# yanzq95/DHD

Hardware: AMD Instinct MI355X
Metric: samples/sec (6-cam fwd+bwd) DHD-S view-transform hot path (higher is better)
Workload: dtype f32

## Files before the change

### dhd_amd/csrc/sfa_gemm_cu.h

```cpp
#pragma once
#include "sfa_math.h"
#include "sfa_mfma.h"

namespace dhd_sfa {

constexpr int kCuPatchPitch = 36;

__device__ __forceinline__ void cu_lds_barrier() { asm volatile("s_waitcnt lgkmcnt(0)\n\ts_barrier" ::: "memory"); }

constexpr int cu_swz_c(int p) { return ((((p >> 2) & 7) ^ (p & 1)) | (((p >> 1) & 1) << 3)); }
__host__ __device__ inline int cu_swz(int p) { return ((((p >> 2) & 7) ^ (p & 1)) | (((p >> 1) & 1) << 3)); }

inline size_t cu_lds_bytes(int c, int waves, int nb, bool blend = false) {
  return (size_t)2 * 2 * 32 * 2 * c + (size_t)waves * 32 * kCuPatchPitch * sizeof(float) + ((size_t)nb * 3 + 1) * c * sizeof(float) +
         (blend ? ((size_t)nb + 2) * c * sizeof(float) : 0);
}
inline int cu_max_batch(int c, int waves, bool blend = false) {
  return (int)((160 * 1024 - cu_lds_bytes(c, waves, 0, blend)) / ((size_t)(blend ? 4 : 3) * c * sizeof(float)));
}

struct CuBlend {
  const void* x;
  const float* a1;
  const float* scsh;
// ... 232 lines not shown
        return;
      }
#pragma unroll
      for (int mt = 0; mt < MT; ++mt) {
        if (NACC == 2) {
          acc2[mt] = mfma_bf16(wm[ks][mt], bh, ks == 0 ? zero : acc2[mt]);
          acc[mt] = mfma_bf16(wh[ks][mt], bh, ks == 0 ? zero : acc[mt]);
          acc2[mt] = mfma_bf16(wh[ks][mt], bm, acc2[mt]);
        } else {
          acc[mt] = mfma_bf16(wm[ks][mt], bh, ks == 0 ? zero : acc[mt]);
          acc[mt] = mfma_bf16(wh[ks][mt], bm, acc[mt]);
          acc[mt] = mfma_bf16(wh[ks][mt], bh, acc[mt]);
        }
      }
    });
    stamp(0);
    if (PP) cu_lds_barrier();
    auto next_tile = [&]() {
    stage(std::integral_constant<int, SN>{}, (PAR ^ 1) ^ grp, t + (1 + grp) * t_step);
    stamp(1);
    issue(std::integral_constant<int, SN>{}, t + (1 + grp + R) * t_step);
    stamp(2);
    };
    auto epilogue = [&]() {
    const __amdgpu_buffer_rsrc_t ry =
        __builtin_amdgcn_make_buffer_rsrc(y + (size_t)b * C * hw, 0, (unsigned)((size_t)C * hw * sizeof(float)), 0x00020000);
    const bool quad_ok = live && p0 + 4 * q < hw;
    const int voff_st = quad_ok ? st_voff : 0x7ffffff0;
    if (ABL & 4) {
#pragma unroll
      for (int mt = 0; mt < MT; ++mt)
#pragma unroll
        for (int v = 0; v < 16; ++v) abl_sink += acc[mt][v] + (NACC == 2 ? acc2[mt][v] : 0.f);
    }
#pragma unroll
    for (int mt = 0; mt < ((ABL & 4) ? 0 : MT); ++mt) {
#pragma unroll
      for (int v = 0; v < 16; ++v)
        patch[(8 * (v >> 2) + 4 * h + (v & 3)) * kCuPatchPitch + n] = NACC == 2 ? acc[mt][v] + acc2[mt][v] : acc[mt][v];
#pragma unroll
      for (int k = 0; k < 4; ++k) {
        f32x4 o = *reinterpret_cast<const f32x4*>(patch + (g + 8 * k) * kCuPatchPitch + 4 * q);
        if (EPI == 0) {
          const float s1 = (o.x + o.y) + (o.z + o.w), s2 = (o.x * o.x + o.y * o.y) + (o.z * o.z + o.w * o.w);
          ws1[mt][k] += quad_ok ? s1 : 0.f;
          ws2[mt][k] += quad_ok ? s2 : 0.f;
          const float bs = bias_lds[kbase + 32 * mt + g + 8 * k];
          o.x += bs; o.y += bs; o.z += bs; o.w += bs;
        }
        if (EPI == 1) {
          const int w4 = (int)(mask_r[mt][k] >> (4 * (g & 3)));
#pragma unroll
          for (int e = 0; e < 4; ++e) o[e] = __int_as_float(__float_as_int(o[e]) & __builtin_amdgcn_sbfe(w4, e, 1));
        }
        const int soff = (32 * mt + 8 * k) * row_bytes + p0 * 4;
        if (EPI == 3) {
          const int ch = kbase + 32 * mt + g + 8 * k;
          const float bs = bias_lds[ch];
          o.x += bs; o.y += bs; o.z += bs; o.w += bs;
          const float a = bl_a[b * C + ch], na = 1.0f - a, sc = bl_sc[ch], sh = bl_sc[C + ch];
          const f32x4 pb = xb[mt][k], pv = xv[mt][k];
          f32x4 r;
#pragma unroll
          for (int j = 0; j < 4; ++j) {
            r[j] = blend_out(blend_gate(sc, o[j], sh), a, na, pb[j], pv[j]);
          }
          const __amdgpu_buffer_rsrc_t ro = __builtin_amdgcn_make_buffer_rsrc(
              static_cast<TO*>(bl.out) + (size_t)b * C * hw, 0, (unsigned)((size_t)C * hw * sizeof(TO)), 0x00020000);
          if constexpr (std::is_same_v<TO, float>) {
            store_b128_guarded<SAUX>(__builtin_bit_cast(u32x4, r), ro, voff_st, soff);
          } else {
            typedef TO t4 __attribute__((ext_vector_type(4)));
            const t4 hv = {(TO)r.x, (TO)r.y, (TO)r.z, (TO)r.w};
            __builtin_amdgcn_raw_buffer_store_b64(__builtin_bit_cast(u32x2, hv), ro, quad_ok ? st_voff >> 1 : 0x7ffffff0, soff >> 1, SAUX);
          }
          continue;
        }
        if (!(ABL & 2)) store_b128_guarded<SAUX>(__builtin_bit_cast(u32x4, o), ry, voff_st, soff);
      }
    }
    };
    if (EORD == 0) { next_tile(); epilogue(); } else { epilogue(); next_tile(); }
    stamp(3);
    cu_lds_barrier();
  };

  if (n_mine > 0) {
    auto fill_stores = [&]() {
      const __amdgpu_buffer_rsrc_t ry = __builtin_amdgcn_make_buffer_rsrc(y, 0, 16, 0x00020000);
#pragma unroll
      for (int i = 0; i < 4 * MT; ++i)
        if (!(ABL & 2)) store_b128_guarded<SAUX>(u32x4{0u, 0u, 0u, 0u}, ry, 0x7ffffff0, 0);
    };
    issue(std::integral_constant<int, 0>{}, t0);
    if (R == 2) {
      issue(std::integral_constant<int, 1 % R>{}, t0 + t_step);
      fill_stores();
    }
    stage(std::integral_constant<int, 0>{}, 0, t0);
    issue(std::integral_constant<int, 0>{}, t0 + R * t_step);
    fill_stores();
    cu_lds_barrier();
    if (PP && grp) {
      stage(std::integral_constant<int, 0>{}, 1, t0 + t_step);
      issue(std::integral_constant<int, 0>{}, t0 + 2 * t_step);
      fill_stores();
      cu_lds_barrier();
    }
    for (int i = 0, t = t0; i < n_mine; i += 2, t += 2 * t_step) {
      tile(std::integral_constant<int, 0>{}, t, true);
      tile(std::integral_constant<int, 1>{}, t + t_step, i + 1 < n_mine);
    }
    if (PP && !grp) cu_lds_barrier();
  }

  if ((ABL & 256) && lane == 0) {
    unsigned* o = reinterpret_cast<unsigned*>(stat_part) + 1024 + ((size_t)blockIdx.x * WAVES + wv) * 8;
    for (int i = 0; i < 6; ++i) o[i] = ph[i];
    o[6] = (unsigned)n_mine;
  }
  if ((ABL & 64) && tid == 0) reinterpret_cast<long long*>(stat_part)[blockIdx.x] = (long long)__builtin_readcyclecounter() - abl_clk0;
  if (EPI == 0 && stat_part != nullptr) {
#pragma unroll
    for (int mt = 0; mt < MT; ++mt)
#pragma unroll
      for (int k = 0; k < 4; ++k) {
        float s1 = ws1[mt][k], s2 = ws2[mt][k];
#pragma unroll
        for (int m = 1; m < 8; m <<= 1) {
          s1 += __shfl_xor(s1, m, DHD_WAVE);
          s2 += __shfl_xor(s2, m, DHD_WAVE);
        }
        if (q == 0) {
          float* row = stat_part + (size_t)blockIdx.x * 2 * C + kbase + 32 * mt + g + 8 * k;
          row[0] = s1;
          row[C] = s2;
        }
      }
  }
}

}
```

### dhd_amd/csrc/sfa_stage.hip

```cpp
#include <stdlib.h>

#include <type_traits>

#include "sfa_gemm_cu.h"
#include "sfa_half.h"
#include "sfa_mfma.h"

using namespace dhd_sfa;

namespace {

constexpr int kEwBlock = 256;
constexpr int kPlaneChunks = 4;
constexpr int kPwBlock = 256;
constexpr int kPwStep = 16;
constexpr int kWgBlock = 512;
constexpr int kWgStride = 33;
constexpr int kWgWorkers = 256;

__device__ __forceinline__ float block_sum(float v, float* sm) {
  v = group_sum(v, DHD_WAVE);
  const int lane = threadIdx.x & 63, wv = threadIdx.x >> 6;
  __syncthreads();
  if (lane == 0) sm[wv] = v;
  __syncthreads();
  float t = 0.f;
  for (int k = 0; k < (int)(blockDim.x / DHD_WAVE); ++k) t += sm[k];
  return t;
}

template <class TS> constexpr bool kHalfStorage = !std::is_same_v<TS, float>;
template <class TS> constexpr bool kStreamAll = kHalfStorage<TS>;
template <class TS> constexpr int kWideInFlight = kHalfStorage<TS> ? 2 : 1;
template <class TS> constexpr bool kFoldPairwise = !kHalfStorage<TS>;

template <int N> __device__ __forceinline__ void chunk_range(int hw, int* lo, int* hi) {
  static_assert(N == 4 || N == 8, "16 bytes of float32 or of a half type");
  const int n = hw >> (N == 8 ? 3 : 2), per = (n + kPlaneChunks - 1) / kPlaneChunks;
  *lo = blockIdx.x * per;
  *hi = min(n, *lo + per);
}

template <class TO, int N> struct IoVec {
  static constexpr bool k16 = N == kVec16<TO>;
  static_assert(k16 || (N == 4 && sizeof(TO) == 2), "16 bytes, or four elements of a half type");
  using raw = std::conditional_t<k16, raw16<TO>, u32x2>;
  static __device__ __forceinline__ raw ld(const TO* base, size_t i) { return __builtin_nontemporal_load(reinterpret_cast<const raw*>(base) + i); }
  static __device__ __forceinline__ void widen(raw w, float* v) {
    if constexpr (k16) {
      widen16<TO>(w, v);
    } else {
      const f32x2 a = Pair<TO>::widen(w.x), b = Pair<TO>::widen(w.y);
      v[0] = a.x; v[1] = a.y; v[2] = b.x; v[3] = b.y;
// ... 40 lines not shown
      body(w, i + kEwBlock);
    }
    if (i < hi) body(load(i), i);
  } else {
    for (; i < hi; i += kEwBlock) body(load(i), i);
  }
}


template <class TS>
__device__ __forceinline__ void plane_mean_block(const TS* __restrict__ x, float* __restrict__ part, int hw, float* sm) {
  constexpr int N = kVec16<TS>;
  using X = Vec16<TS, true>;
  const size_t plane = blockIdx.y;
  const TS* p = x + plane * hw;
  int lo, hi;
  chunk_range<N>(hw, &lo, &hi);
  float a0 = 0.f, a1 = 0.f;
  int i = lo + threadIdx.x;
  for (; i + kEwBlock < hi; i += 2 * kEwBlock) {
    float v[N], w[N];
    X::load(p, i, v);
    X::load(p, (size_t)i + kEwBlock, w);
    a0 += tree_sum<N>(v);
    a1 += tree_sum<N>(w);
  }
  if (i < hi) {
    float v[N];
    X::load(p, i, v);
    a0 += tree_sum<N>(v);
  }
  const float tot = block_sum(a0 + a1, sm);
  if (threadIdx.x == 0) part[plane * kPlaneChunks + blockIdx.x] = tot;
}

__global__ __launch_bounds__(kEwBlock) void plane_mean_kernel(const float* __restrict__ x, float* __restrict__ part, int hw) {
  __shared__ float sm[kEwBlock / DHD_WAVE];
  plane_mean_block(x, part, hw, sm);
}

constexpr int kFcBlock = 1024;
__global__ __launch_bounds__(kFcBlock) void fc_forward_kernel(const float* __restrict__ part, const float* __restrict__ w1,
                                                              const float* __restrict__ b1, const float* __restrict__ w2,
                                                              const float* __restrict__ b2, float* __restrict__ s,
                                                              float* __restrict__ hbuf, float* __restrict__ a,
                                                              float* __restrict__ tab, int c, int r, int hw,
                                                              int* __restrict__ ticks, int n_ticks) {
  extern __shared__ float sh[];
  if (blockIdx.x == 0)
    for (int i = threadIdx.x; i < n_ticks; i += kFcBlock) ticks[i] = 0;
  float* ss = sh;
  float* hh = sh + 2 * c;
  const int b = blockIdx.x, c2 = 2 * c;
  for (int i = threadIdx.x; i < c2; i += kFcBlock) {
    const float* q = part + ((size_t)b * c2 + i) * kPlaneChunks;
    float v = ((q[0] + q[1]) + (q[2] + q[3])) / (float)hw;
    ss[i] = v;
    s[(size_t)b * c2 + i] = v;
  }
  __syncthreads();
  const int lane = threadIdx.x & 63, wv = threadIdx.x >> 6;
  for (int j0 = wv * 4; j0 < r; j0 += 4 * (kFcBlock / DHD_WAVE)) {
    float acc[4] = {0.f, 0.f, 0.f, 0.f};
    for (int i = lane; i < c2; i += DHD_WAVE) {
      const float sv = ss[i];
#pragma unroll
      for (int q = 0; q < 4; ++q)
        if (j0 + q < r) acc[q] = fmaf(w1[(size_t)(j0 + q) * c2 + i], sv, acc[q]);
    }
#pragma unroll
    for (int q = 0; q < 4; ++q) {
      const float t = group_sum(acc[q], DHD_WAVE);
      if (lane == 0 && j0 + q < r) {
        const float v = fmaxf(t + b1[j0 + q], 0.f);
        hh[j0 + q] = v;
        hbuf[(size_t)b * r + j0 + q] = v;
      }
    }
  }
  __syncthreads();
  for (int k = threadIdx.x; k < c; k += kFcBlock) {
    float acc = b2[k];
    if ((r & 3) == 0) {
      const f32x4* wrow = reinterpret_cast<const f32x4*>(w2 + (size_t)k * r);
#pragma unroll 8
      for (int j = 0; j < (r >> 2); ++j) {
        const f32x4 wv4 = wrow[j];
        acc = fmaf(wv4.x, hh[4 * j], acc);
        acc = fmaf(wv4.y, hh[4 * j + 1], acc);
        acc = fmaf(wv4.z, hh[4 * j + 2], acc);
        acc = fmaf(wv4.w, hh[4 * j + 3], acc);
      }
    } else {
      for (int j = 0; j < r; ++j) acc = fmaf(w2[(size_t)k * r + j], hh[j], acc);
    }
    float v = sigmoidf_(acc);
    a[(size_t)b * c + k] = v;
    float* t = tab + (size_t)b * 3 * c;
    t[k] = v;
    t[c + k] = 1.0f - v;
    t[2 * c + k] = 0.f;
  }
}

__global__ __launch_bounds__(kEwBlock) void fc_backward_kernel(const float* __restrict__ da_p1, const float* __restrict__ da_p2,
                                                               const float* __restrict__ a, const float* __restrict__ hbuf,
                                                               const float* __restrict__ w1, const float* __restrict__ w2,
                                                               float* __restrict__ dpre2, float* __restrict__ dh,
                                                               float* __restrict__ ds, int c, int r) {
  extern __shared__ float sh[];
  float* sp = sh;
  float* sd = sh + c;
  const int b = blockIdx.x, c2 = 2 * c;
  for (int k = threadIdx.x; k < c; k += kEwBlock) {
    float g = 0.f;
    for (int q = 0; q < kPlaneChunks; ++q)
      g += da_p1[((size_t)b * kPlaneChunks + q) * c + k] + da_p2[((size_t)b * kPlaneChunks + q) * c + k];
    const float av = a[(size_t)b * c + k];
    const float v = g * av * (1.0f - av);
    sp[k] = v;
    dpre2[(size_t)b * c + k] = v;
  }
  __syncthreads();
  if (r <= kEwBlock && kEwBlock % r == 0) {
    float* pp = sh + c + r;
    const int groups = kEwBlock / r, j = threadIdx.x % r, grp = threadIdx.x / r;
    float acc = 0.f;
#pragma unroll 8
    for (int k = grp; k < c; k += groups) acc = fmaf(w2[(size_t)k * r + j], sp[k], acc);
    pp[grp * r + j] = acc;
    __syncthreads();
    if (threadIdx.x < r) {
      float t = 0.f;
      for (int q = 0; q < groups; ++q) t += pp[q * r + threadIdx.x];
      const float v = hbuf[(size_t)b * r + threadIdx.x] > 0.f ? t : 0.f;
      sd[threadIdx.x] = v;
// ... 125 lines not shown
  scsh[c + ch] = shf;
  for (int b = 0; b < nb; ++b) {
    float* t = tab + (size_t)b * 3 * c;
    t[ch] = sc;
    t[c + ch] = 0.f;
    t[2 * c + ch] = shf;
  }
  if (run_mean) {
    const double unb = n > 1.0 ? var * n / (n - 1.0) : var;
    run_mean[ch] = (float)((1.0 - (double)momentum) * (double)run_mean[ch] + (double)momentum * mu);
    run_var[ch] = (float)((1.0 - (double)momentum) * (double)run_var[ch] + (double)momentum * unb);
  }
}

__device__ __forceinline__ void bn_eval_coef_channel(int ch, const float* __restrict__ gamma, const float* __restrict__ beta,
                                                     const float* __restrict__ run_mean, const float* __restrict__ run_var, float eps,
                                                     float* __restrict__ mean, float* __restrict__ rstd, float* __restrict__ scsh,
                                                     float* __restrict__ tab, int nb, int c) {
  const float rs = 1.0f / sqrtf(run_var[ch] + eps);
  mean[ch] = run_mean[ch];
  rstd[ch] = rs;
  const float sc = gamma[ch] * rs, shf = beta[ch] - run_mean[ch] * sc;
  scsh[ch] = sc;
  scsh[c + ch] = shf;
  for (int b = 0; b < nb; ++b) {
    float* t = tab + (size_t)b * 3 * c;
    t[ch] = sc;
    t[c + ch] = 0.f;
    t[2 * c + ch] = shf;
  }
}

__global__ __launch_bounds__(kEwBlock) void bn_eval_coef_kernel(const float* __restrict__ gamma, const float* __restrict__ beta,
                                                                const float* __restrict__ run_mean, const float* __restrict__ run_var,
                                                                float eps, float* __restrict__ mean, float* __restrict__ rstd,
                                                                float* __restrict__ scsh, float* __restrict__ tab, int nb, int c) {
  const int ch = blockIdx.x * kEwBlock + threadIdx.x;
  if (ch >= c) return;
  bn_eval_coef_channel(ch, gamma, beta, run_mean, run_var, eps, mean, rstd, scsh, tab, nb, c);
}

struct BnEvalJob {
  const float *gamma, *beta, *run_mean, *run_var;
  float eps;
  float *mean, *rstd, *scsh, *tab;
};
__global__ __launch_bounds__(kEwBlock) void bn_eval_coef2_kernel(BnEvalJob j1, BnEvalJob j2, int nb, int c) {
  const int ch = blockIdx.x * kEwBlock + threadIdx.x;
  if (ch >= c) return;
  const BnEvalJob& j = blockIdx.y ? j2 : j1;
  bn_eval_coef_channel(ch, j.gamma, j.beta, j.run_mean, j.run_var, j.eps, j.mean, j.rstd, j.scsh, j.tab, nb, c);
}

template <bool COHERENT>
__device__ __forceinline__ void bn_backward_coef_channel(const float* __restrict__ part, int ch, const float* __restrict__ gamma,
                                                         const float* __restrict__ mean, const float* __restrict__ rstd,
                                                         int training, float* __restrict__ tab, float* __restrict__ dgamma,
                                                         float* __restrict__ dbeta, float* __restrict__ dbias, int nb, int c, int hw,
                                                         double* __restrict__ sums_out, const double* __restrict__ sums_in,
                                                         const double* __restrict__ loc_fwd, const float* __restrict__ shift) {
  double s1 = 0.0, s2 = 0.0;
  if (COHERENT) {
    float v1[16], v2[16];
    for (int q0 = 0; q0 < nb * kPlaneChunks; q0 += 16) {
#pragma unroll
      for (int u = 0; u < 16; ++u) {
        const int q = min(q0 + u, nb * kPlaneChunks - 1);
        v1[u] = __hip_atomic_load(part + ((size_t)q * 2) * c + ch, __ATOMIC_RELAXED, __HIP_MEMORY_SCOPE_AGENT);
        v2[u] = __hip_atomic_load(part + ((size_t)q * 2 + 1) * c + ch, __ATOMIC_RELAXED, __HIP_MEMORY_SCOPE_AGENT);
      }
#pragma unroll
      for (int u = 0; u < 16; ++u)
        if (q0 + u < nb * kPlaneChunks) { s1 += (double)v1[u]; s2 += (double)v2[u]; }
    }
  } else {
    for (int q = 0; q < nb * kPlaneChunks; ++q) {
      s1 += (double)part[((size_t)q * 2) * c + ch];
      s2 += (double)part[((size_t)q * 2 + 1) * c + ch];
    }
  }
  const double n_loc = (double)nb * (double)hw;
  if (sums_out) {
    sums_out[ch] = s1; sums_out[c + ch] = s2;
    if (ch == 0) sums_out[2 * c] = n_loc;
    return;
  }
  const double n = sums_in ? sums_in[2 * c] : n_loc;
  const double g1 = sums_in ? sums_in[ch] : s1, g2 = sums_in ? sums_in[c + ch] : s2;
  const double rs = (double)rstd[ch], mu = (double)mean[ch], ga = (double)gamma[ch];
  if (dgamma) dgamma[ch] = (float)(rs * s2);
  if (dbeta) dbeta[ch] = (float)s1;
  double c0 = ga * rs, c1 = 0.0, c2 = 0.0, db = c0 * s1;
  if (training) {
    c1 = -ga * rs * rs * rs * g2 / n;
    c2 = -ga * rs * g1 / n - c1 * mu;
    db = 0.0;
    if (sums_in) db = c0 * s1 + c1 * (loc_fwd[ch] + n_loc * (double)shift[ch]) + n_loc * c2;
  }
  if (dbias) dbias[ch] = (float)db;
  for (int b = 0; b < nb; ++b) {
    float* t = tab + (size_t)b * 3 * c;
    t[ch] = (float)c0;
    t[c + ch] = (float)c1;
    t[2 * c + ch] = (float)c2;
  }
}

__global__ __launch_bounds__(kEwBlock) void bn_backward_coef_kernel(const float* __restrict__ part, const float* __restrict__ gamma,
                                                                    const float* __restrict__ mean, const float* __restrict__ rstd,
                                                                    int training, float* __restrict__ tab, float* __restrict__ dgamma,
                                                                    float* __restrict__ dbeta, float* __restrict__ dbias, int nb,
                                                                    int c, int hw, double* __restrict__ sums_out,
                                                                    const double* __restrict__ sums_in, const double* __restrict__ loc_fwd,
                                                                    const float* __restrict__ shift) {
  const int ch = blockIdx.x * kEwBlock + threadIdx.x;
  if (ch >= c) return;
  bn_backward_coef_channel<false>(part, ch, gamma, mean, rstd, training, tab, dgamma, dbeta, dbias, nb, c, hw, sums_out, sums_in,
                                  loc_fwd, shift);
}

struct BnTail {
  int* ticket;
  const float* gamma;
  const float* mean;
  const float* rstd;
  float* tab;
  float* dgamma;
  float* dbeta;
  float* dbias;
  int training, nb, hw;
};
__device__ __forceinline__ void bn_backward_publish(const BnTail& t, float* __restrict__ part, size_t q, int ch, int c, float s1,
                                                    float s2) {
  float* p1 = part + (q * 2) * c + ch;
  float* p2 = part + (q * 2 + 1) * c + ch;
  if (t.ticket == nullptr) {
    *p1 = s1;
    *p2 = s2;
    return;
  }
  __hip_atomic_store(p1, s1, __ATOMIC_RELAXED, __HIP_MEMORY_SCOPE_AGENT);
  __hip_atomic_store(p2, s2, __ATOMIC_RELAXED, __HIP_MEMORY_SCOPE_AGENT);
  asm volatile("s_waitcnt vmcnt(0)" ::: "memory");
  if (__hip_atomic_fetch_add(t.ticket + ch, 1, __ATOMIC_RELAXED, __HIP_MEMORY_SCOPE_AGENT) != t.nb * kPlaneChunks - 1) return;
  __hip_atomic_store(t.ticket + ch, 0, __ATOMIC_RELAXED, __HIP_MEMORY_SCOPE_AGENT);
  bn_backward_coef_channel<true>(part, ch, t.gamma, t.mean, t.rstd, t.training, t.tab, t.dgamma, t.dbeta, t.dbias, t.nb, c, t.hw,
                                 nullptr, nullptr, nullptr, nullptr);
}

template <class TS>
__global__ __launch_bounds__(kEwBlock) void pair_sums_kernel(const TS* __restrict__ g, const TS* __restrict__ y,
                                                             const float* __restrict__ mean, float* __restrict__ part, int c, int hw,
                                                             BnTail tail) {
  constexpr int N = kVec16<TS>;
  using Main = Vec16<TS, true>;
  using Tail = Vec16<TS, kStreamAll<TS>>;
  __shared__ float sm[kEwBlock / DHD_WAVE];
  const int plane = blockIdx.y, b = plane / c, ch = plane % c;
  const float mu = mean[ch];
  const TS* gp = g + (size_t)plane * hw;
  const TS* yp = y + (size_t)plane * hw;
  int lo, hi;
  chunk_range<N>(hw, &lo, &hi);
  float s1 = 0.f, s2 = 0.f, t1 = 0.f, t2 = 0.f;
  int i = lo + threadIdx.x;
  for (; i + kEwBlock < hi; i += 2 * kEwBlock) {
    float a[N], v[N], a2[N], v2[N];
    Main::load(gp, i, a);
    Main::load(yp, i, v);
    Main::load(gp, (size_t)i + kEwBlock, a2);
    Main::load(yp, (size_t)i + kEwBlock, v2);
    s1 = fold_sum<TS>(s1, a);
    s2 = fold_dot<TS>(s2, a, [&](int j) { return v[j] - mu; });
    t1 = fold_sum<TS>(t1, a2);
    t2 = fold_dot<TS>(t2, a2, [&](int j) { return v2[j] - mu; });
  }
  if (i < hi) {
    float a[N], v[N];
    Tail::load(gp, i, a);
    Tail::load(yp, i, v);
    s1 = fold_sum<TS>(s1, a);
    s2 = fold_dot<TS>(s2, a, [&](int j) { return v[j] - mu; });
  }
  s1 = block_sum(s1 + t1, sm);
  s2 = block_sum(s2 + t2, sm);
  if (threadIdx.x == 0) bn_backward_publish(tail, part, (size_t)(b * kPlaneChunks + blockIdx.x), ch, c, s1, s2);
}


template <class TS, class TO>
__global__ __launch_bounds__(kEwBlock) void blend2_bn_kernel(const TS* __restrict__ x, const float* __restrict__ a1,
                                                             const TS* __restrict__ y2, const float* __restrict__ scsh,
                                                             TO* __restrict__ out, int c, int hw) {
  constexpr int N = kVec16<TS>;
  using X = Vec16<TS, true>;
  using Y2 = Vec16<TS, kStreamAll<TS>>;
  const int plane = blockIdx.y, b = plane / c, ch = plane % c;
  const float a = a1[plane], na = 1.0f - a, sc = scsh[ch], sh = scsh[c + ch];
  const TS* xb = x + ((size_t)b * 2 * c + ch) * hw;
  const TS* xv = x + ((size_t)b * 2 * c + c + ch) * hw;
  const TS* yp = y2 + (size_t)plane * hw;
  TO* op = out + (size_t)plane * hw;
  int lo, hi;
  chunk_range<N>(hw, &lo, &hi);
  for (int i = lo + threadIdx.x; i < hi; i += kEwBlock) {
    float p[N], q[N], s[N], r[N];
    X::load(xb, i, p);
    X::load(xv, i, q);
    Y2::load(yp, i, s);
#pragma unroll
    for (int j = 0; j < N; ++j) r[j] = blend_out(blend_gate(sc, s[j], sh), a, na, p[j], q[j]);
    IoVec<TO, N>::store(op, i, r);
  }
}

template <class TS, class TO>
__global__ __launch_bounds__(kEwBlock) void blend2_bn_bwd_kernel(const TS* __restrict__ x, const float* __restrict__ a1,
                                                                 const TS* __restrict__ y2, const float* __restrict__ scsh,
                                                                 const float* __restrict__ mean, const TO* __restrict__ go,
                                                                 TS* __restrict__ g2, float* __restrict__ part,
                                                                 float* __restrict__ da_p1, int c, int hw, BnTail tail) {
  constexpr int N = kVec16<TS>;
  using X = Vec16<TS, true>;
  using Y2 = Vec16<TS, kStreamAll<TS>>;
  using G2 = Vec16<TS, kStreamAll<TS>>;
  using Go = IoVec<TO, N>;
  __shared__ float sm[kEwBlock / DHD_WAVE];
  const int plane = blockIdx.y, b = plane / c, ch = plane % c;
  const float a = a1[plane], na = 1.0f - a, sc = scsh[ch], sh = scsh[c + ch], mu = mean[ch];
  const TS* xb = x + ((size_t)b * 2 * c + ch) * hw;
  const TS* xv = x + ((size_t)b * 2 * c + c + ch) * hw;
  const TS* yp = y2 + (size_t)plane * hw;
  const TO* gp = go + (size_t)plane * hw;
  TS* rp = g2 + (size_t)plane * hw;
  int lo, hi;
  chunk_range<N>(hw, &lo, &hi);
  float s1 = 0.f, s2 = 0.f, sa = 0.f;
  struct In {
    raw16<TS> p, q, s;
// ... 448 lines not shown
  L.wpart = f((size_t)kWgWorkers * cc);
  L.total = o;
  return L;
}

inline int device_index() {
  int d = 0;
  (void)hipGetDevice(&d);
  return d < 0 || d >= 64 ? 0 : d;
}

int cu_count() {
  static int n[64] = {};
  const int dev = device_index();
  if (n[dev] == 0 && hipDeviceGetAttribute(&n[dev], hipDeviceAttributeMultiprocessorCount, dev) != hipSuccess) n[dev] = -1;
  return n[dev];
}

template <auto Kern>
int lds_limit_once(size_t bytes) {
  static bool done[64] = {};
  const int dev = device_index();
  if (!done[dev]) {
    DHD_HIP(hipFuncSetAttribute(reinterpret_cast<const void*>(Kern), hipFuncAttributeMaxDynamicSharedMemorySize, (int)bytes));
    done[dev] = true;
  }
  return DHD_OK;
}
template <auto Kern, class... Args>
int launch_lds(dim3 grid, dim3 block, size_t shmem, size_t limit, hipStream_t st, Args... args) {
  if (int rc = lds_limit_once<Kern>(limit); rc != DHD_OK) return rc;
  hipLaunchKernelGGL(Kern, grid, block, shmem, st, args...);
  DHD_LAUNCH_CHECK();
  return DHD_OK;
}

inline int res_cob(int c, int nt) {
  for (int cob = 4; cob >= 1; cob >>= 1)
    if (32 * cob <= c && (size_t)(c / 16) * cob * nt * 1024 <= kResWeightMax) return cob;
  return 0;
}

enum class Gemm { cu, cuh, res, streamed6, f32 };
enum class Wgrad { w3, w6, f32, half };
enum class Pack { cu, res, six, f32, cuh };
struct Plan {
  int storage;
  Gemm gemm;
  Wgrad wgrad;
  Pack pack;
  int nt, cob;
  int cot;
  bool fused_stats;
};

int make_plan(const dhd_sfa_weights* w, int c, int hw, Plan* p) {
  *p = Plan{};
  switch (w->gemm) {
    case DHD_SFA_GEMM_DEFAULT: case DHD_SFA_GEMM_BF16X3: p->nt = 2; break;
    case DHD_SFA_GEMM_BF16X6: p->nt = 3; break;
    case DHD_SFA_GEMM_F32: p->nt = 0; break;
    default: return DHD_EINVAL;
  }
  if (w->io_dtype != DHD_F32 && w->io_dtype != DHD_F16 && w->io_dtype != DHD_BF16) return DHD_EINVAL;
  p->storage = w->storage_dtype;
  if (p->storage != DHD_F32) {
    if (p->storage != DHD_F16 && p->storage != DHD_BF16) return DHD_EINVAL;
    if (w->io_dtype != p->storage) return DHD_EINVAL;
    if (!half_storage_supported(c, hw)) return DHD_EUNSUPPORTED;
    p->gemm = Gemm::cuh; p->wgrad = Wgrad::half; p->pack = Pack::cuh;
    p->fused_stats = w->training != 0;
    return DHD_OK;
  }
  p->fused_stats = w->training && p->nt > 0;
  p->cob = p->nt > 0 ? res_cob(c, p->nt) : 0;
  p->cot = c % 256 == 0 ? 8 : 4;
  p->wgrad = p->nt == 2 ? Wgrad::w3 : p->nt == 3 ? Wgrad::w6 : Wgrad::f32;
  if (p->nt == 2 && (c == 128 || c == 256)) {
    p->gemm = Gemm::cu; p->pack = Pack::cu;
  } else if ((p->nt == 2 && c == 512) || (p->nt == 3 && c <= 256)) {
    p->gemm = Gemm::res; p->pack = Pack::res;
  } else if (p->nt > 0) {
    p->gemm = Gemm::streamed6; p->pack = Pack::six;
  } else {
    p->gemm = Gemm::f32; p->pack = Pack::f32;
  }
  return DHD_OK;
}

enum Op { kConv1, kConv2, kDgrad2, kDgrad1, kConv2Blend };
template <int OP>
struct Variant {
  static constexpr bool two = OP != kConv2 && OP != kConv2Blend;
  static constexpr bool relu = OP == kConv2 || OP == kConv2Blend;
  static constexpr int epi = OP == kDgrad2 ? 1 : OP == kDgrad1 ? 2 : OP == kConv2Blend ? 3 : 0;
  static constexpr bool rec = OP == kConv2;
};
template <class F>
int with_op(Op op, F&& f) {
  switch (op) {
    case kConv1: return f(Variant<kConv1>{});
    case kConv2: return f(Variant<kConv2>{});
    case kDgrad2: return f(Variant<kDgrad2>{});
    case kDgrad1: return f(Variant<kDgrad1>{});
    case kConv2Blend: return f(Variant<kConv2Blend>{});
  }
  return DHD_EUNSUPPORTED;
}

template <class TS>
struct GemmCall {
  Op op;
  const TS* in0;
  const TS* in1;
  size_t in_bstride;
  int in_channels;
  const float* coef;
  const void* wp;
  const float* bias;
  unsigned* mask;
  float* stat_part;
  TS* y;
  const TS* aux;
  const float* aux_scsh;
  CuBlend blend;
  int out_dtype;
};

template <class TS>
int launch_gemm_cu(const GemmCall<TS>& g, int b, int c, int hw, hipStream_t st, int* stat_rows) {
  constexpr bool kHalf = !std::is_same<TS, float>::value;
  const int waves = c / 32;
// ... 312 lines not shown
  if (hi <= 1) return DHD_OK;
  coef(bn2, y2, TF(T.tab_g2));
  hipLaunchKernelGGL((blend2_bn_kernel<TS, TO>), planes, dim3(kEwBlock), 0, st, x, SF(S.a1), y2, SF(S.scsh2), out, c, hw);
  DHD_LAUNCH_CHECK();
  return DHD_OK;
}

template <class TS, class TO>
int stage_backward(const Plan& p, const TS* x, const dhd_sfa_weights* w, const void* saved, const TO* gout, TO* gx,
                   const dhd_sfa_grads* grads, void* scratch, int b, int c, int hw, int lo, int hi, double* sync, hipStream_t st) {
  const int r = w->hidden;
  const SavedLayout S = saved_layout(b, c, hw, r, p.storage);
  const ScratchLayout T = scratch_layout(b, c, hw, r, p.storage);
  char* sv = const_cast<char*>(static_cast<const char*>(saved));
  char* sc = static_cast<char*>(scratch);
  auto SF = [&](size_t off) { return reinterpret_cast<float*>(sv + off); };
  auto TF = [&](size_t off) { return reinterpret_cast<float*>(sc + off); };
  const TS* y1 = reinterpret_cast<const TS*>(sv + S.y1);
  const TS* y2 = reinterpret_cast<const TS*>(sv + S.y2);
  TS* g2 = reinterpret_cast<TS*>(sc + T.g2);
  TS* g1 = reinterpret_cast<TS*>(sc + T.g1);
  TS* du = reinterpret_cast<TS*>(sc + T.du);
  unsigned* mask = reinterpret_cast<unsigned*>(sv + S.mask);
  int* tick = reinterpret_cast<int*>(sv + S.tick);
  const dim3 planes(kPlaneChunks, b * c), per_ch(dhd_cdiv(c, kEwBlock));
  const size_t cs = (size_t)c * hw;
  int rc;
  const BnTail tail2 = {sync ? nullptr : tick, w->bn2_w, SF(S.mean2), SF(S.rstd2), TF(T.tab_g2), grads->bn2_w, grads->bn2_b,
                        grads->conv2_b, w->training, b, hw};
  const BnTail tail1 = {sync ? nullptr : tick + c, w->bn1_w, SF(S.mean1), SF(S.rstd1), TF(T.tab_g1), grads->bn1_w, grads->bn1_b,
                        grads->conv1_b, w->training, b, hw};
  auto coef_out = [&](const BnTail& t) {
    hipLaunchKernelGGL(bn_backward_coef_kernel, per_ch, dim3(kEwBlock), 0, st, TF(T.part), t.gamma, t.mean, t.rstd, w->training, t.tab,
                       t.dgamma, t.dbeta, t.dbias, b, c, hw, sync, nullptr, nullptr, nullptr);
  };
  auto coef_in = [&](const BnTail& t, size_t loc, const float* bias) {
    hipLaunchKernelGGL(bn_backward_coef_kernel, per_ch, dim3(kEwBlock), 0, st, TF(T.part), t.gamma, t.mean, t.rstd, w->training, t.tab,
                       t.dgamma, t.dbeta, t.dbias, b, c, hw, nullptr, sync, reinterpret_cast<const double*>(sv + loc), bias);
  };
  if (sync && !p.fused_stats) return DHD_EUNSUPPORTED;

  if (lo <= 0) {
    hipLaunchKernelGGL((blend2_bn_bwd_kernel<TS, TO>), planes, dim3(kEwBlock), 0, st, x, SF(S.a1), y2, SF(S.scsh2), SF(S.mean2), gout, g2, TF(T.part),
                       TF(T.da1), c, hw, tail2);
    if (sync) coef_out(tail2);
    DHD_LAUNCH_CHECK();
  }
  if (hi <= 0) return DHD_OK;
  if (lo <= 1) {
    if (sync) coef_in(tail2, S.loc2, w->conv2_b);
    DHD_LAUNCH_CHECK();
    rc = launch_wgrad<TS>(p, kConv2, g2, y2, TF(T.tab_g2), cs, y1, nullptr, SF(S.tab1), cs, TF(T.wpart), grads->conv2_w, b, c, hw, st);
    if (rc != DHD_OK) return rc;
    rc = launch_gemm(p, GemmCall<TS>{kDgrad2, g2, y2, cs, c, TF(T.tab_g2), sv + S.wp2t, nullptr, mask, nullptr, g1, y1, SF(S.scsh1)},
                     b, c, hw, st);
    if (rc != DHD_OK) return rc;
    hipLaunchKernelGGL(pair_sums_kernel<TS>, planes, dim3(kEwBlock), 0, st, g1, y1, SF(S.mean1), TF(T.part), c, hw, tail1);
    if (sync) coef_out(tail1);
    DHD_LAUNCH_CHECK();
  }
  if (hi <= 1) return DHD_OK;
  if (sync) coef_in(tail1, S.loc1, w->conv1_b);
  DHD_LAUNCH_CHECK();
  rc = launch_wgrad<TS>(p, kConv1, g1, y1, TF(T.tab_g1), cs, x, x + cs, SF(S.tab_a), 2 * cs, TF(T.wpart), grads->conv1_w, b, c, hw, st);
  if (rc != DHD_OK) return rc;
  rc = launch_gemm(p, GemmCall<TS>{kDgrad1, g1, y1, cs, c, TF(T.tab_g1), sv + S.wp1t, nullptr, nullptr, nullptr, du}, b, c, hw, st);
  if (rc != DHD_OK) return rc;
  hipLaunchKernelGGL(blend1_da_kernel<TS>, planes, dim3(kEwBlock), 0, st, x, du, TF(T.da2), c, hw);
  hipLaunchKernelGGL(fc_backward_kernel, dim3(b), dim3(kEwBlock), (size_t)(c + r + kEwBlock) * sizeof(float), st, TF(T.da1), TF(T.da2),
                     SF(S.a1), SF(S.h), w->fc1_w, w->fc2_w, TF(T.dpre2), TF(T.dh), TF(T.ds), c, r);
  const int n_fc = r * 2 * c + c * r + r + c;
  const FcGradJob fcj = {TF(T.dpre2), TF(T.dh), SF(S.h), SF(S.s), grads->fc1_w, grads->fc1_b, grads->fc2_w, grads->fc2_b, b, r};
  const int fc_rows = dhd_cdiv(dhd_cdiv(n_fc, kEwBlock), kPlaneChunks);
  const dim3 planes_fc(kPlaneChunks, b * c + fc_rows);
  hipLaunchKernelGGL((stage_gx_kernel<TS, TO>), planes_fc, dim3(kEwBlock), 0, st, SF(S.a1), y2, SF(S.scsh2), gout, du, TF(T.ds), gx, c, hw, fc_rows, fcj);
  DHD_LAUNCH_CHECK();
  return DHD_OK;
}

inline bool infer_form_exists(const Plan& p, int form) {
  switch (form) {
    case DHD_SFA_INFER_AUTO: case DHD_SFA_INFER_UNFUSED: return true;
    case DHD_SFA_INFER_TWO_PASS: return p.gemm == Gemm::cu || p.gemm == Gemm::cuh;
    case DHD_SFA_INFER_ONE_PASS: return p.gemm == Gemm::cuh;
    default: return false;
  }
}
inline int infer_resolve(const Plan& p, int form) {
  if (form != DHD_SFA_INFER_AUTO) return form;
  if (infer_form_exists(p, DHD_SFA_INFER_ONE_PASS)) return DHD_SFA_INFER_ONE_PASS;
  return infer_form_exists(p, DHD_SFA_INFER_TWO_PASS) ? DHD_SFA_INFER_TWO_PASS : DHD_SFA_INFER_UNFUSED;
}

struct InferLayout {
  size_t wp1, wp2, mean_part, s, h, a1, tab_a, mean1, rstd1, scsh1, tab1, mean2, rstd2, scsh2, tab2, y1, total;
};
inline InferLayout infer_layout(int b, int c, int hw, int r, int storage, bool with_y1) {
  const bool half = storage != DHD_F32;
  const size_t cc = (size_t)c * c;
  InferLayout L;
  size_t o = 0;
  auto take = [&](size_t bytes) { size_t at = o; o += (bytes + 255) & ~(size_t)255; return at; };
  auto f = [&](size_t n) { return take(n * sizeof(float)); };
  L.wp1 = take(half ? 2 * cc : 8 * cc); L.wp2 = take(half ? 2 * cc : 8 * cc);
  L.mean_part = f((size_t)b * 2 * c * kPlaneChunks);
  L.s = f((size_t)b * 2 * c); L.h = f((size_t)b * r); L.a1 = f((size_t)b * c); L.tab_a = f((size_t)b * 3 * c);
  L.mean1 = f(c); L.rstd1 = f(c); L.scsh1 = f(2 * c); L.tab1 = f((size_t)b * 3 * c);
  L.mean2 = f(c); L.rstd2 = f(c); L.scsh2 = f(2 * c); L.tab2 = f((size_t)b * 3 * c);
  L.y1 = take(with_y1 ? (size_t)b * c * hw * (half ? 2 : 4) : 0);
  L.total = o;
// ... 222 lines not shown
```

Measured before the change: 2568.

## Derive BN1 backward sums from conv2 weight grad instead of streaming activations

In the backward pass, BN1's statistics are now computed from a different source. The gradient sum comes from per-tile sums fused into the dgrad2 GEMM epilogue, and the gradient·(y−mean) sum is recovered algebraically from sum_k w2·dw2 via the ReLU/affine identity. This replaces the pair_sums pass over g1 and y1. A fallback streaming path is kept for channels where |beta| is large relative to gamma, and an env var can select the old behaviour. Separately, the FC forward kernel preloads its small weight matrices into registers. The identity trades a full activation read for possible numerical error, which a new script checks.

```diff
diff --git a/dhd_amd/csrc/sfa_gemm_cu.h b/dhd_amd/csrc/sfa_gemm_cu.h
--- a/dhd_amd/csrc/sfa_gemm_cu.h
+++ b/dhd_amd/csrc/sfa_gemm_cu.h
@@ -308,6 +308,7 @@
           const int w4 = (int)(mask_r[mt][k] >> (4 * (g & 3)));
 #pragma unroll
           for (int e = 0; e < 4; ++e) o[e] = __int_as_float(__float_as_int(o[e]) & __builtin_amdgcn_sbfe(w4, e, 1));
+          ws1[mt][k] += quad_ok ? (o.x + o.y) + (o.z + o.w) : 0.f;
         }
         const int soff = (32 * mt + 8 * k) * row_bytes + p0 * 4;
         if (EPI == 3) {
@@ -376,7 +377,7 @@
     o[6] = (unsigned)n_mine;
   }
   if ((ABL & 64) && tid == 0) reinterpret_cast<long long*>(stat_part)[blockIdx.x] = (long long)__builtin_readcyclecounter() - abl_clk0;
-  if (EPI == 0 && stat_part != nullptr) {
+  if ((EPI == 0 || EPI == 1) && stat_part != nullptr) {
 #pragma unroll
     for (int mt = 0; mt < MT; ++mt)
 #pragma unroll
@@ -390,7 +391,7 @@
         if (q == 0) {
           float* row = stat_part + (size_t)blockIdx.x * 2 * C + kbase + 32 * mt + g + 8 * k;
           row[0] = s1;
-          row[C] = s2;
+          if (EPI == 0) row[C] = s2;
         }
       }
   }
diff --git a/dhd_amd/csrc/sfa_stage.hip b/dhd_amd/csrc/sfa_stage.hip
--- a/dhd_amd/csrc/sfa_stage.hip
+++ b/dhd_amd/csrc/sfa_stage.hip
@@ -1,4 +1,5 @@
 #include <stdlib.h>
+#include <string.h>
 
 #include <type_traits>
 
@@ -145,6 +146,22 @@
   float* ss = sh;
   float* hh = sh + 2 * c;
   const int b = blockIdx.x, c2 = 2 * c;
+  const int lane = threadIdx.x & 63, wv = threadIdx.x >> 6;
+  const bool pre = c2 <= 8 * DHD_WAVE && r <= 32 && (r & 3) == 0 && c <= kFcBlock;
+  float w1r[4][8];
+  f32x4 w2r[8];
+  if (pre) {
+#pragma unroll
+    for (int q = 0; q < 4; ++q)
+#pragma unroll
+      for (int e = 0; e < 8; ++e) {
+        const int i = lane + DHD_WAVE * e;
+        w1r[q][e] = (wv * 4 + q < r && i < c2) ? w1[(size_t)(wv * 4 + q) * c2 + i] : 0.f;
+      }
+#pragma unroll
+    for (int j = 0; j < 8; ++j)
+      w2r[j] = ((int)threadIdx.x < c && 4 * j < r) ? reinterpret_cast<const f32x4*>(w2 + (size_t)threadIdx.x * r)[j] : f32x4{0.f, 0.f, 0.f, 0.f};
+  }
   for (int i = threadIdx.x; i < c2; i += kFcBlock) {
     const float* q = part + ((size_t)b * c2 + i) * kPlaneChunks;
     float v = ((q[0] + q[1]) + (q[2] + q[3])) / (float)hw;
@@ -152,14 +169,26 @@
     s[(size_t)b * c2 + i] = v;
   }
   __syncthreads();
-  const int lane = threadIdx.x & 63, wv = threadIdx.x >> 6;
   for (int j0 = wv * 4; j0 < r; j0 += 4 * (kFcBlock / DHD_WAVE)) {
     float acc[4] = {0.f, 0.f, 0.f, 0.f};
-    for (int i = lane; i < c2; i += DHD_WAVE) {
-      const float sv = ss[i];
-#pragma unroll
-      for (int q = 0; q < 4; ++q)
-        if (j0 + q < r) acc[q] = fmaf(w1[(size_t)(j0 + q) * c2 + i], sv, acc[q]);
+    if (pre) {
+#pragma unroll
+      for (int e = 0; e < 8; ++e) {
+        const int i = lane + DHD_WAVE * e;
+        if (i < c2) {
+          const float sv = ss[i];
+#pragma unroll
+          for (int q = 0; q < 4; ++q)
+            if (j0 + q < r) acc[q] = fmaf(w1r[q][e], sv, acc[q]);
+        }
+      }
+    } else {
+      for (int i = lane; i < c2; i += DHD_WAVE) {
+        const float sv = ss[i];
+#pragma unroll
+        for (int q = 0; q < 4; ++q)
+          if (j0 + q < r) acc[q] = fmaf(w1[(size_t)(j0 + q) * c2 + i], sv, acc[q]);
+      }
     }
 #pragma unroll
     for (int q = 0; q < 4; ++q) {
@@ -174,7 +203,16 @@
   __syncthreads();
   for (int k = threadIdx.x; k < c; k += kFcBlock) {
     float acc = b2[k];
-    if ((r & 3) == 0) {
+    if (pre) {
+#pragma unroll
+      for (int j = 0; j < 8; ++j)
+        if (4 * j < r) {
+          acc = fmaf(w2r[j].x, hh[4 * j], acc);
+          acc = fmaf(w2r[j].y, hh[4 * j + 1], acc);
+          acc = fmaf(w2r[j].z, hh[4 * j + 2], acc);
+          acc = fmaf(w2r[j].w, hh[4 * j + 3], acc);
+        }
+    } else if ((r & 3) == 0) {
       const f32x4* wrow = reinterpret_cast<const f32x4*>(w2 + (size_t)k * r);
 #pragma unroll 8
       for (int j = 0; j < (r >> 2); ++j) {
@@ -406,6 +444,39 @@
   bn_eval_coef_channel(ch, j.gamma, j.beta, j.run_mean, j.run_var, j.eps, j.mean, j.rstd, j.scsh, j.tab, nb, c);
 }
 
+__device__ __forceinline__ void bn_backward_coef_apply(double s1, double s2, int ch, const float* __restrict__ gamma,
+                                                       const float* __restrict__ mean, const float* __restrict__ rstd, int training,
+                                                       float* __restrict__ tab, float* __restrict__ dgamma, float* __restrict__ dbeta,
+                                                       float* __restrict__ dbias, int nb, int c, int hw,
+                                                       double* __restrict__ sums_out, const double* __restrict__ sums_in,
+                                                       const double* __restrict__ loc_fwd, const float* __restrict__ shift) {
+  const double n_loc = (double)nb * (double)hw;
+  if (sums_out) {
+    sums_out[ch] = s1; sums_out[c + ch] = s2;
+    if (ch == 0) sums_out[2 * c] = n_loc;
+    return;
+  }
+  const double n = sums_in ? sums_in[2 * c] : n_loc;
+  const double g1 = sums_in ? sums_in[ch] : s1, g2 = sums_in ? sums_in[c + ch] : s2;
+  const double rs = (double)rstd[ch], mu = (double)mean[ch], ga = (double)gamma[ch];
+  if (dgamma) dgamma[ch] = (float)(rs * s2);
+  if (dbeta) dbeta[ch] = (float)s1;
+  double c0 = ga * rs, c1 = 0.0, c2 = 0.0, db = c0 * s1;
+  if (training) {
+    c1 = -ga * rs * rs * rs * g2 / n;
+    c2 = -ga * rs * g1 / n - c1 * mu;
+    db = 0.0;
+    if (sums_in) db = c0 * s1 + c1 * (loc_fwd[ch] + n_loc * (double)shift[ch]) + n_loc * c2;
+  }
+  if (dbias) dbias[ch] = (float)db;
+  for (int b = 0; b < nb; ++b) {
+    float* t = tab + (size_t)b * 3 * c;
+    t[ch] = (float)c0;
+    t[c + ch] = (float)c1;
+    t[2 * c + ch] = (float)c2;
+  }
+}
+
 template <bool COHERENT>
 __device__ __forceinline__ void bn_backward_coef_channel(const float* __restrict__ part, int ch, const float* __restrict__ gamma,
                                                          const float* __restrict__ mean, const float* __restrict__ rstd,
@@ -433,31 +504,8 @@
       s2 += (double)part[((size_t)q * 2 + 1) * c + ch];
     }
   }
-  const double n_loc = (double)nb * (double)hw;
-  if (sums_out) {
-    sums_out[ch] = s1; sums_out[c + ch] = s2;
-    if (ch == 0) sums_out[2 * c] = n_loc;
-    return;
-  }
-  const double n = sums_in ? sums_in[2 * c] : n_loc;
-  const double g1 = sums_in ? sums_in[ch] : s1, g2 = sums_in ? sums_in[c + ch] : s2;
-  const double rs = (double)rstd[ch], mu = (double)mean[ch], ga = (double)gamma[ch];
-  if (dgamma) dgamma[ch] = (float)(rs * s2);
-  if (dbeta) dbeta[ch] = (float)s1;
-  double c0 = ga * rs, c1 = 0.0, c2 = 0.0, db = c0 * s1;
-  if (training) {
-    c1 = -ga * rs * rs * rs * g2 / n;
-    c2 = -ga * rs * g1 / n - c1 * mu;
-    db = 0.0;
-    if (sums_in) db = c0 * s1 + c1 * (loc_fwd[ch] + n_loc * (double)shift[ch]) + n_loc * c2;
-  }
-  if (dbias) dbias[ch] = (float)db;
-  for (int b = 0; b < nb; ++b) {
-    float* t = tab + (size_t)b * 3 * c;
-    t[ch] = (float)c0;
-    t[c + ch] = (float)c1;
-    t[2 * c + ch] = (float)c2;
-  }
+  bn_backward_coef_apply(s1, s2, ch, gamma, mean, rstd, training, tab, dgamma, dbeta, dbias, nb, c, hw, sums_out, sums_in, loc_fwd,
+                         shift);
 }
 
 __global__ __launch_bounds__(kEwBlock) void bn_backward_coef_kernel(const float* __restrict__ part, const float* __restrict__ gamma,
@@ -539,6 +587,67 @@
   s1 = block_sum(s1 + t1, sm);
   s2 = block_sum(s2 + t2, sm);
   if (threadIdx.x == 0) bn_backward_publish(tail, part, (size_t)(b * kPlaneChunks + blockIdx.x), ch, c, s1, s2);
+}
+
+constexpr int kBn1Block = 1024;
+constexpr float kBn1Rho = 0.25f;
+__global__ __launch_bounds__(kBn1Block) void bn1_backward_from_dw2_kernel(const float* __restrict__ stat, int n_rows,
+                                                                          const float* __restrict__ w2, const float* __restrict__ dw2,
+                                                                          const float* __restrict__ beta, const float* __restrict__ scsh,
+                                                                          const float* __restrict__ g, const float* __restrict__ y,
+                                                                          int force_stream, int c, int hw, BnTail tail) {
+  using Main = Vec16<float, true>;
+  __shared__ double sm[kBn1Block / DHD_WAVE][2];
+  const int nblk = gridDim.x, t = threadIdx.x;
+  const int ch = (nblk & 7) == 0 ? (blockIdx.x & 7) * (nblk >> 3) + (blockIdx.x >> 3) : blockIdx.x;
+  const float sc = scsh[ch], be = beta[ch], mu = tail.mean[ch];
+  const bool ident = !force_stream && fabsf(be) <= kBn1Rho * fabsf(tail.gamma[ch]) && sc != 0.f && __builtin_isfinite(sc);
+  double a1 = 0.0, a2 = 0.0;
+  if (ident) {
+    for (int i = t; i < n_rows; i += kBn1Block) a1 += (double)stat[(size_t)i * 2 * c + ch];
+    for (int k = t; k < c; k += kBn1Block) a2 += (double)w2[(size_t)k * c + ch] * (double)dw2[(size_t)k * c + ch];
+  } else {
+    const int n = hw >> 2;
+    float s1 = 0.f, s2 = 0.f, t1 = 0.f, t2 = 0.f;
+    for (int b = 0; b < tail.nb; ++b) {
+      const float* gp = g + ((size_t)b * c + ch) * hw;
+      const float* yp = y + ((size_t)b * c + ch) * hw;
+      int i = t;
+      for (; i + kBn1Block < n; i += 2 * kBn1Block) {
+        float a[4], v[4], a2v[4], v2[4];
+        Main::load(gp, i, a);
+        Main::load(yp, i, v);
+        Main::load(gp, (size_t)i + kBn1Block, a2v);
+        Main::load(yp, (size_t)i + kBn1Block, v2);
+        s1 = fold_sum<float>(s1, a);
+        s2 = fold_dot<float>(s2, a, [&](int j) { return v[j] - mu; });
+        t1 = fold_sum<float>(t1, a2v);
+        t2 = fold_dot<float>(t2, a2v, [&](int j) { return v2[j] - mu; });
+      }
+      if (i < n) {
+        float a[4], v[4];
+        Main::load(gp, i, a);
+        Main::load(yp, i, v);
+        s1 = fold_sum<float>(s1, a);
+        s2 = fold_dot<float>(s2, a, [&](int j) { return v[j] - mu; });
+      }
+    }
+    a1 = (double)s1 + (double)t1;
+    a2 = (double)s2 + (double)t2;
+  }
+#pragma unroll
+  for (int m = DHD_WAVE / 2; m > 0; m >>= 1) {
+    a1 += __shfl_xor(a1, m, DHD_WAVE);
+    a2 += __shfl_xor(a2, m, DHD_WAVE);
+  }
+  if ((t & (DHD_WAVE - 1)) == 0) { sm[t / DHD_WAVE][0] = a1; sm[t / DHD_WAVE][1] = a2; }
+  __syncthreads();
+  if (t != 0) return;
+  a1 = a2 = 0.0;
+  for (int k = 0; k < kBn1Block / DHD_WAVE; ++k) { a1 += sm[k][0]; a2 += sm[k][1]; }
+  if (ident) a2 = (a2 - (double)be * a1) / (double)sc;
+  bn_backward_coef_apply(a1, a2, ch, tail.gamma, tail.mean, tail.rstd, tail.training, tail.tab, tail.dgamma, tail.dbeta, tail.dbias,
+                         tail.nb, c, tail.hw, nullptr, nullptr, nullptr, nullptr);
 }
 
 
@@ -1093,6 +1202,7 @@
   int nt, cob;
   int cot;
   bool fused_stats;
+  bool bn1_from_dw2, bn1_stream;
 };
 
 int make_plan(const dhd_sfa_weights* w, int c, int hw, Plan* p) {
@@ -1119,6 +1229,10 @@
   p->wgrad = p->nt == 2 ? Wgrad::w3 : p->nt == 3 ? Wgrad::w6 : Wgrad::f32;
   if (p->nt == 2 && (c == 128 || c == 256)) {
     p->gemm = Gemm::cu; p->pack = Pack::cu;
+    const char* e = getenv("DHD_SFA_BN1_SUMS");
+    if (e && *e && strcmp(e, "auto") != 0 && strcmp(e, "pair_sums") != 0 && strcmp(e, "stream") != 0) return DHD_EINVAL;
+    p->bn1_from_dw2 = !(e && strcmp(e, "pair_sums") == 0);
+    p->bn1_stream = e && strcmp(e, "stream") == 0;
   } else if ((p->nt == 2 && c == 512) || (p->nt == 3 && c <= 256)) {
     p->gemm = Gemm::res; p->pack = Pack::res;
   } else if (p->nt > 0) {
@@ -1537,10 +1651,18 @@
     DHD_LAUNCH_CHECK();
     rc = launch_wgrad<TS>(p, kConv2, g2, y2, TF(T.tab_g2), cs, y1, nullptr, SF(S.tab1), cs, TF(T.wpart), grads->conv2_w, b, c, hw, st);
     if (rc != DHD_OK) return rc;
-    rc = launch_gemm(p, GemmCall<TS>{kDgrad2, g2, y2, cs, c, TF(T.tab_g2), sv + S.wp2t, nullptr, mask, nullptr, g1, y1, SF(S.scsh1)},
-                     b, c, hw, st);
+    const bool from_dw2 = std::is_same<TS, float>::value && p.bn1_from_dw2 && !sync;
+    int stat_rows = 0;
+    rc = launch_gemm(p, GemmCall<TS>{kDgrad2, g2, y2, cs, c, TF(T.tab_g2), sv + S.wp2t, nullptr, mask, from_dw2 ? TF(T.stat_part) : nullptr,
+                                     g1, y1, SF(S.scsh1)},
+                     b, c, hw, st, &stat_rows);
     if (rc != DHD_OK) return rc;
-    hipLaunchKernelGGL(pair_sums_kernel<TS>, planes, dim3(kEwBlock), 0, st, g1, y1, SF(S.mean1), TF(T.part), c, hw, tail1);
+    if constexpr (std::is_same<TS, float>::value) {
+      if (from_dw2)
+        hipLaunchKernelGGL(bn1_backward_from_dw2_kernel, dim3(c), dim3(kBn1Block), 0, st, TF(T.stat_part), stat_rows, w->conv2_w,
+                           grads->conv2_w, w->bn1_b, SF(S.scsh1), g1, y1, p.bn1_stream ? 1 : 0, c, hw, tail1);
+    }
+    if (!from_dw2) hipLaunchKernelGGL(pair_sums_kernel<TS>, planes, dim3(kEwBlock), 0, st, g1, y1, SF(S.mean1), TF(T.part), c, hw, tail1);
     if (sync) coef_out(tail1);
     DHD_LAUNCH_CHECK();
   }
diff --git a/experiments/sfa_bn1_identity_check.py b/experiments/sfa_bn1_identity_check.py
--- /dev/null
+++ b/experiments/sfa_bn1_identity_check.py
@@ -0,0 +1,74 @@
+import sys
+
+import torch
+
+
+def split(x):
+    h = x.float().bfloat16().float()
+    m = (x.float() - h).bfloat16().float()
+    return h.double(), m.double()
+
+
+def mm3(a, b):
+    ah, am = split(a)
+    bh, bm = split(b)
+    return (ah @ bh + ah @ bm + am @ bh).float().double()
+
+
+def case(c, b, hw, gamma, beta, seed):
+    g = torch.Generator().manual_seed(seed)
+    p = b * hw
+    y1 = (torch.randn(c, p, generator=g) * (0.5 + torch.rand(c, 1, generator=g)) + torch.randn(c, 1, generator=g)).float()
+    mu = y1.double().mean(1).float()
+    var = y1.double().var(1, unbiased=False)
+    rstd = (1.0 / torch.sqrt(var + 1e-5)).float()
+    sc = (gamma * rstd).float()
+    sh = (beta - mu * sc).float()
+    pre = torch.addcmul(sh[:, None], sc[:, None], y1).float()
+    mask = pre > 0
+    z1 = pre * mask
+    w2 = (torch.randn(c, c, generator=g) / c ** 0.5).float()
+    dy2 = torch.randn(c, p, generator=g).float()
+    d = (y1 - mu[:, None]).float()
+    g1x = mask * (w2.double().t() @ dy2.double())
+    s2x = (g1x * (y1.double() - mu.double()[:, None])).sum(1)
+    g1 = (mask * mm3(w2.t(), dy2)).float()
+    s1 = g1.sum(1)
+    s2p = (g1 * d).sum(1).double()
+    dw2 = mm3(dy2, z1.t())
+    sz = (w2.double() * dw2).sum(0)
+    s2i = (sz - beta.double() * s1.double()) / sc.double()
+    scale = s2x.abs().max()
+    return [((s - s2x).abs().max() / scale).item() for s in (s2p, s2i)]
+
+
+def params(c, seed, kind, rho):
+    g = torch.Generator().manual_seed(1000 + seed)
+    gamma = 0.5 + torch.rand(c, generator=g)
+    sign = torch.where(torch.rand(c, generator=g) < 0.5, -1.0, 1.0)
+    if kind == 'typical':
+        beta = torch.rand(c, generator=g) - 0.5
+    else:
+        beta = sign * rho * gamma
+    return gamma.float(), beta.float()
+
+
+def main():
+    shapes = [(128, 3, 1440), (256, 2, 3120)]
+    seeds = [0, 1, 2]
+    print('%-28s %-16s %10s %10s %7s' % ('case', '(C, B, hw)', 'parent', 'identity', 'ratio'))
+    rows = [('typical', 0.0)] + [('boundary', r) for r in (0.25, 0.5, 1.0, 2.0, 4.0)]
+    for kind, rho in rows:
+        for shp in shapes:
+            worst = [0.0, 0.0]
+            for s in seeds:
+                ga, be = params(shp[0], s, kind, rho)
+                e = case(*shp, ga, be, s)
+                worst = [max(a, b) for a, b in zip(worst, e)]
+            name = 'gamma U(.5,1.5), beta U(-.5,.5)' if kind == 'typical' else '|beta| = %g |gamma|' % rho
+            print('%-28s %-16s %10.2e %10.2e %7.2f' % (name[:28], shp, worst[0], worst[1], worst[1] / worst[0]))
+            sys.stdout.flush()
+
+
+if __name__ == '__main__':
+    main()
```

Result: no change. 2565 (-0.1%).
